# akio-tomiya/LatticeQCD.jl

Measured on AMD Instinct MI355X. Metric: CG iters/sec (D^+D) & Dslash GFLOP/s, 32^3x64 SU(3) Wilson fp64, higher is better.
Workload: dtype f64; 1 GPU; configs[3]: 32x32x32x64 Wilson D^+D CG (fixed-length window), fp64; dslash_variant=1, xcd_remap=2, xcd_nsub=16, xcd_ysplit=4, cg_fused=3, gauge_recon=12, gauge_recon_active=1, comm_backend=none, comm_requested=auto

## Files before the change

### latticeqcd.jl_amd/csrc/blas.hip

```cpp
#include "lqcd_internal.h"

#include <cstring>

namespace lqcd {

constexpr int RB = 256;

__device__ inline void block_reduce2(double a, double b, double* partial, int stride) {
    __shared__ double red[2][RB / 64];
#pragma unroll
    for (int off = 32; off > 0; off >>= 1) { a += __shfl_down(a, off, 64); b += __shfl_down(b, off, 64); }
    if ((threadIdx.x & 63) == 0) { red[0][threadIdx.x >> 6] = a; red[1][threadIdx.x >> 6] = b; }
    __syncthreads();
    if (threadIdx.x == 0) {
        double sa = 0, sb = 0;
#pragma unroll
        for (int w = 0; w < RB / 64; w++) { sa += red[0][w]; sb += red[1][w]; }
        partial[blockIdx.x * stride] = sa;
        if (stride > 1) partial[blockIdx.x * stride + 1] = sb;
    }
}

__global__ __launch_bounds__(RB) void dot_kernel(const double2* __restrict__ a, const double2* __restrict__ b, size_t n,
                                                 double* partial) {
    double re = 0, im = 0;
    for (size_t i = (size_t)blockIdx.x * RB + threadIdx.x; i < n; i += (size_t)gridDim.x * RB) {
        const double2 x = a[i], y = b[i];
        re = fma(x.x, y.x, re); re = fma(x.y, y.y, re);
        im = fma(x.x, y.y, im); im = fma(-x.y, y.x, im);
    }
    block_reduce2(re, im, partial, 2);
}

__global__ __launch_bounds__(RB) void norm2_kernel(const double2* __restrict__ a, size_t n, double* partial) {
    double s = 0;
    for (size_t i = (size_t)blockIdx.x * RB + threadIdx.x; i < n; i += (size_t)gridDim.x * RB) {
        const double2 x = a[i];
        s = fma(x.x, x.x, s); s = fma(x.y, x.y, s);
    }
    block_reduce2(s, 0.0, partial, 1);
}

__global__ __launch_bounds__(FB) void reduce_final(const double* __restrict__ partial, int nblocks, int nvals, double* scal, int slot, int op, PeerRedArgs pr, int soa) {
    __shared__ double tot[PEER_RED_VALS];
    if (nblocks <= 1024) {
        if (threadIdx.x < 64) {
            double mine = 0.0;
            for (int v = 0; v < nvals; v++) {
                const double t = sum_partials_small_nv(partial, nblocks, nvals, v, soa != 0);
                if (pr.nranks) { if (((int)threadIdx.x >> 3) == v) mine = t; }
                else if (threadIdx.x == 0) scal[slot + v] = t;
            }
            if (pr.nranks) {
                const double s = peer_allreduce_wave(pr, mine, nvals);
                for (int q = 0; q < nvals; q++) {
                    const double v = __shfl(s, 8 * q, 64);
                    if (threadIdx.x == 0) scal[slot + q] = v;
                }
            }
            if (op && threadIdx.x == 0) cg_scalar_step(scal, op);
        }
        return;
    }
    __shared__ double redv[PEER_RED_VALS][FB / 64];
    double cls[PEER_RED_VALS];
#pragma unroll
    for (int v = 0; v < PEER_RED_VALS; v++)
        if (v < nvals) cls[v] = sum_partials_class(partial, nblocks, nvals, v, (int)threadIdx.x, soa != 0);
#pragma unroll
    for (int v = 0; v < PEER_RED_VALS; v++)
        if (v < nvals) {
            const double w = shfl_tree_sum(cls[v]);
            if ((threadIdx.x & 63) == 0) redv[v][threadIdx.x >> 6] = w;
        }
    __syncthreads();
    if ((int)threadIdx.x < nvals) {
        double t = 0;
        for (int w = 0; w < FB / 64; w++) t += redv[threadIdx.x][w];
        if (pr.nranks) tot[threadIdx.x] = t; else scal[slot + threadIdx.x] = t;
    }
    __syncthreads();
    if (pr.nranks && threadIdx.x < 64) {
        const int k = (int)threadIdx.x >> 3;
        const double s = peer_allreduce_wave(pr, k < nvals ? tot[k] : 0.0, nvals);
        for (int q = 0; q < nvals; q++) {
            const double v = __shfl(s, 8 * q, 64);
            if (threadIdx.x == 0) scal[slot + q] = v;
        }
    }
    if (op && threadIdx.x == 0) cg_scalar_step(scal, op);
}

__global__ __launch_bounds__(RB) void axpy_kernel(double ar, double ai, const double2* __restrict__ x, double2* __restrict__ y, size_t n) {
    for (size_t i = (size_t)blockIdx.x * RB + threadIdx.x; i < n; i += (size_t)gridDim.x * RB) {
        const double2 xv = x[i];
        double2 yv = y[i];
        yv.x = fma(ar, xv.x, yv.x); yv.x = fma(-ai, xv.y, yv.x);
        yv.y = fma(ar, xv.y, yv.y); yv.y = fma(ai, xv.x, yv.y);
        y[i] = yv;
    }
}

__global__ __launch_bounds__(RB) void axpby_kernel(double ar, double ai, const double2* __restrict__ x, double br, double bi,
// ... 25 lines not shown
int allreduce_host(lqcd_ctx_s* c, double* vals, int n) {
    if (!c->has_comm) return LQCD_OK;
    ARGCHK(n <= 8, "allreduce_host: too many values");
    double* d = c->d_scal + SCAL_DOUBLES - 8;
    HIPCHK(hipMemcpyAsync(d, vals, n * sizeof(double), hipMemcpyHostToDevice, c->stream));
    LQCHK(comm_allreduce(c, d, n));
    HIPCHK(hipMemcpyAsync(vals, d, n * sizeof(double), hipMemcpyDeviceToHost, c->stream));
    HIPCHK(hipStreamSynchronize(c->stream));
    return comm_check(c);
}

int reduce_tail(lqcd_ctx_s* c, int nvals, int slot, int cg_op) {
    if (c->has_comm || cg_op) return comm_allreduce(c, c->d_scal + slot, nvals, cg_op);
    return LQCD_OK;
}

int reduce_to_slot(lqcd_ctx_s* c, int nblocks, int nvals, int slot, bool allreduce, int cg_op, const double* partial, bool soa) {
    const bool multi = allreduce && c->has_comm;
    const bool peer = multi && c->peer.on;
    ARGCHK(nvals >= 1 && nvals <= PEER_RED_VALS, "reduce_to_slot: one to eight values per reduction");
    if (peer) ARGCHK(nvals <= PEER_RED_VALS, "reduce_to_slot: more than 8 values in one reduction over the ranks");
    PeerRedArgs pr;
    if (peer) pr = comm_red_args(c); else memset(&pr, 0, sizeof pr);
    hipLaunchKernelGGL(reduce_final, dim3(1), dim3(FB), 0, c->stream, partial ? partial : c->d_partial, nblocks, nvals, c->d_scal, slot, (multi && !peer) ? 0 : cg_op, pr, soa ? 1 : 0);
    HIPCHK(hipGetLastError());
    if (multi && !peer) LQCHK(comm_allreduce(c, c->d_scal + slot, nvals, cg_op));
    return LQCD_OK;
}

int reduce_pack_to_slot(lqcd_ctx_s* c, int nblocks, int slot, int cg_op) {
    if (!c->has_waiting_pack) return reduce_to_slot(c, nblocks, 1, slot, true, cg_op);
    c->has_waiting_pack = false;
    const bool multi = c->has_comm, peer = multi && c->peer.on;
    LQCHK(launch_pack_reduce(c, *static_cast<StencilCall*>(c->waiting_pack), c->d_partial, nblocks, slot, (multi && !peer) ? 0 : cg_op));
    if (multi && !peer) LQCHK(comm_allreduce(c, c->d_scal + slot, 1, cg_op));
    return LQCD_OK;
}

static int fetch_slot(lqcd_ctx_s* c, int slot, int nvals, double* out) {
    HIPCHK(hipMemcpyAsync(c->h_scal, c->d_scal + slot, nvals * sizeof(double), hipMemcpyDeviceToHost, c->stream));
    HIPCHK(hipStreamSynchronize(c->stream));
    for (int i = 0; i < nvals; i++) out[i] = c->h_scal[i];
    return LQCD_OK;
}

int blas_dot(lqcd_ctx_s* c, const double2* a, const double2* b, size_t n, double* re, double* im, bool allreduce) {
    HIPCHK(hipSetDevice(c->device));
// ... 74 lines not shown
```

### latticeqcd.jl_amd/csrc/capi.hip

```cpp
#include "lqcd_internal.h"

#include <algorithm>
#include <cstdio>
#include <cstdlib>
#include <cstring>
#include <mutex>

namespace lqcd {

static thread_local std::string g_err;
static std::mutex g_live_mu;
static std::vector<const lqcd_ctx_s*> g_live;
bool ctx_is_live(const lqcd_ctx_s* c) {
    std::lock_guard<std::mutex> lk(g_live_mu);
    for (const lqcd_ctx_s* p : g_live)
        if (p == c) return true;
    return false;
}
static void ctx_set_live(const lqcd_ctx_s* c, bool live) {
    std::lock_guard<std::mutex> lk(g_live_mu);
    for (size_t i = 0; i < g_live.size(); i++)
        if (g_live[i] == c) { g_live.erase(g_live.begin() + i); break; }
    if (live) g_live.push_back(c);
}
// ... 155 lines not shown
    ARGCHK(V / 2 < (1ll << 31) / 16, "lqcd_ctx_create: local volume too large for 32-bit site indices");
    lqcd_ctx_s* c = new lqcd_ctx_s;
    c->home_thread = std::this_thread::get_id();
    c->device = device;
    c->rank = rank;
    c->nranks = pe[0] * pe[1] * pe[2] * pe[3];
    geom_from_L(c->geom, L);
    for (int mu = 0; mu < 4; mu++) {
        c->gL[mu] = gL[mu]; c->pe[mu] = pe[mu]; c->coord[mu] = coord[mu];
        c->nbr_fwd[mu] = nf[mu]; c->nbr_bwd[mu] = nb[mu];
        c->geom.gL[mu] = gL[mu]; c->geom.origin[mu] = origin[mu];
        c->geom.part[mu] = pe[mu] > 1 ? 1 : 0;
    }
    if (const char* e = getenv("LQCD_FORCE_PARTITION")) {
        const int mask = atoi(e);
        for (int mu = 0; mu < 4; mu++)
            if ((mask >> mu) & 1) c->geom.part[mu] = 1;
    }
    {
        const Geom& g = c->geom;
        const long slice = (long)g.XH * g.L[1] * g.L[2];
        if (slice % 64 == 0 && slice / 64 <= 128) { c->tun.xcd_nsub = 8; c->tun.xcd_ysplit = 2; }
        if (gauge12_elems(g) * sizeof(double2) <= ((size_t)256 << 20)) c->tun.nt_gauge = 0;
        if ((size_t)24 * g.Vh * sizeof(double2) <= ((size_t)64 << 20)) c->tun.nt_store = 0;
    }
    if (const char* e = getenv("LQCD_HALO_STREAM_MODE")) {
        const int v = atoi(e);
        if (v < -1 || v > 4) { set_error(std::string("LQCD_HALO_STREAM_MODE=") + e + ": the halo schedule is -1 (timed once) or 0..4"); delete c; return LQCD_ERR_ARG; }
        c->tun.halo_stream_mode = v;
    }
    if (const char* e = getenv("LQCD_HALO_FOLD")) {
        const int v = atoi(e);
        if (v != 0 && v != 1) { set_error(std::string("LQCD_HALO_FOLD=") + e + ": 0 or 1"); delete c; return LQCD_ERR_ARG; }
        c->tun.halo_fold = v;
    }
    hipDeviceProp_t prop;
    HIPCHK(hipGetDeviceProperties(&prop, device));
    c->num_cu = prop.multiProcessorCount > 0 ? prop.multiProcessorCount : 256;
    HIPCHK(hipStreamCreateWithFlags(&c->stream, hipStreamNonBlocking));
    HIPCHK(hipStreamCreateWithFlags(&c->comm_stream, hipStreamNonBlocking));
    HIPCHK(hipEventCreateWithFlags(&c->ev_pack, hipEventDisableTiming));
    HIPCHK(hipEventCreateWithFlags(&c->ev_comm, hipEventDisableTiming));
    HIPCHK(hipEventCreate(&c->ev_t0));
    HIPCHK(hipEventCreate(&c->ev_t1));
    HIPCHK(hipEventCreate(&c->ev_tune0));
    HIPCHK(hipEventCreate(&c->ev_tune1));
    const size_t npart = (size_t)2 * c->geom.Vh / 64 + 4096 + 8 * ((size_t)2 * c->geom.Vh / 128 + 8);
// ... 49 lines not shown
    (void)hipEventDestroy(c->ev_pack); (void)hipEventDestroy(c->ev_comm); (void)hipEventDestroy(c->ev_t0); (void)hipEventDestroy(c->ev_t1);
    (void)hipEventDestroy(c->ev_tune0); (void)hipEventDestroy(c->ev_tune1);
    (void)hipStreamDestroy(c->stream); (void)hipStreamDestroy(c->comm_stream);
    delete c;
    return LQCD_OK;
}

extern "C" int lqcd_ctx_sync(lqcd_ctx_t c) {
    ARGCHK(c, "lqcd_ctx_sync: null");
    LQCHK(ctx_drain_parked(c));
    LQCHK(links_flush_of(c));
    HIPCHK(hipSetDevice(c->device));
    HIPCHK(hipStreamSynchronize(c->stream));
    HIPCHK(hipStreamSynchronize(c->comm_stream));
    return comm_check(c);
}

static int* param_ptr(lqcd_ctx_s* c, const char* key) {
    if (!strcmp(key, "dslash_block")) return &c->tun.dslash_block;
    if (!strcmp(key, "xcd_remap")) return &c->tun.xcd_remap;
    if (!strcmp(key, "dslash_variant")) return &c->tun.dslash_variant;
    if (!strcmp(key, "nt_gauge")) return &c->tun.nt_gauge;
    if (!strcmp(key, "nt_store")) return &c->tun.nt_store;
    if (!strcmp(key, "cg_fused")) return &c->tun.cg_fused;
    if (!strcmp(key, "graph")) return &c->tun.graph;
    if (!strcmp(key, "gauge_recon")) return &c->tun.gauge_recon;
    if (!strcmp(key, "mixed_action_solver")) return &c->tun.mixed_action_solver;
    if (!strcmp(key, "mixed_pair32")) return &c->tun.mixed_pair32;
    if (!strcmp(key, "mixed_links16")) return &c->tun.mixed_links16;
    if (!strcmp(key, "bicg_reliable")) return &c->tun.bicg_reliable;
    if (!strcmp(key, "bicg_rec_guard")) return &c->tun.bicg_rec_guard;
    if (!strcmp(key, "bicg_dot_soa")) return &c->tun.bicg_dot_soa;
    if (!strcmp(key, "clover_hop_s")) return &c->tun.clover_hop_s;
    if (!strcmp(key, "mixed_lean_residual")) return &c->tun.mixed_lean_residual;
    if (!strcmp(key, "mixed_xfuse")) return &c->tun.mixed_xfuse;
    if (!strcmp(key, "mixed_defer_x")) return &c->tun.mixed_defer_x;
    if (!strcmp(key, "pair32_active")) return &c->tun.pair32_active;
    if (!strcmp(key, "stag_both")) return &c->tun.stag_both;
    if (!strcmp(key, "clover_fused")) return &c->tun.clover_fused;
    if (!strcmp(key, "clover_transport")) return &c->tun.clover_transport;
    if (!strcmp(key, "halo_stream_mode")) return &c->tun.halo_stream_mode;
    if (!strcmp(key, "cg_skip_done")) return &c->tun.cg_skip_done;
    if (!strcmp(key, "cg_small")) return &c->tun.cg_small;
    if (!strcmp(key, "cg_tgauge")) return &c->tun.cg_tgauge;
    if (!strcmp(key, "tgauge_active")) return &c->tun.tgauge_active;
    if (!strcmp(key, "cg_sweep_alt")) return &c->tun.cg_sweep_alt;
// ... 198 lines not shown
```

### latticeqcd.jl_amd/csrc/cg.hip

```cpp
#include "ops_internal.h"
#include "stencil_common.h"

#include <algorithm>
#include <cmath>

namespace lqcd {


__global__ void cg_scalar_alpha(double* s) {
    if (s[S_DONE] != 0.0) { s[S_XDONE] = 1.0; return; }
    s[S_ALPHA] = s[S_RR] / s[S_PQ];
}
__global__ void cg_scalar_beta(double* s) {
    if (s[S_DONE] != 0.0) return;
    const double rrn = s[S_RRNEW];
    s[S_BETA] = rrn / s[S_RR];
    s[S_RR] = rrn;
    s[S_ITERS] += 1.0;
    if (rrn < s[S_EPS]) s[S_DONE] = 1.0;
}

__global__ __launch_bounds__(UB) void cg_update_xr(const double* __restrict__ s, double2* __restrict__ x, double2* __restrict__ r,
                                                    const double2* __restrict__ p, const double2* __restrict__ q, size_t n,
                                                    double* partial) {
// ... 444 lines not shown
        apply_bc(c, op->bc);
        LQCHK(make_full_call(op, w.tmp, w.p, 0, s1));
        s1.skip_flag = c->tun.cg_skip_done ? c->d_scal : nullptr;
    } else {
        apply_bc(c, op->bc);
        LQCHK(make_full_call(op, w.tmp, rk, 0, s1));
        s1.upd_scal = c->d_scal;
        s1.upd[0] = spinor_block(w.tmp, 0);
        s1.upd[1] = spinor_block(w.tmp, 1);
        s1.upd_rec = 1;
    }
    s1.gauge12t = gt;
    s1.norm_partial = c->d_partial;
    LQCHK(stencil_apply(c, s1));
    LQCHK(reduce_to_slot(c, nbs, 1, S_PQ, true, m == 0 ? 9 : 7));
    apply_bc(c, op->bc);
    StencilCall s2;
    LQCHK(make_full_call(op, rn, w.tmp, 1, s2));
    s2.gauge12t = gt;
    s2.sweep_rev = w.sweep_alt ? 1 : 0;
    s2.norm_partial = c->d_partial;
    s2.upd_scal = c->d_scal;
    for (int q = 0; q < 2; q++) { s2.upd[q] = spinor_block(rn, q); s2.upd_src[q] = spinor_block(rk, q); }
    LQCHK(stencil_apply(c, s2));
    LQCHK(reduce_to_slot(c, nbs, 1, S_RRNEW, true, 8));
    w.k++;
    return LQCD_OK;
}
static int cg_rring_wanted(lqcd_op_s* op, const CgWork& w) {
    lqcd_ctx_s* c = op->ctx;
    const int K = c->tun.cg_rring;
    if (c->tun.cg_fused < 3 || !(K == 2 || K == 4 || K == 8)) return 0;
    if (op->kind != LQCD_WILSON || op->r != 1.0 || op->csw != 0.0 || any_partitioned(c) || c->has_comm || !c->local_peers.empty()) return 0;
    if (!stencil_sdir_applies(c, op->kind, op->r, op_fused_clover(op))) return 0;
    StencilCall s;
    if (make_full_call(op, w.tmp, w.p, 0, s) != LQCD_OK) return 0;
    if (!(w.tgauge || s.gauge12 || c->tun.dslash_s18)) return 0;
    return K;
}


static int cg_plain_tail(lqcd_ctx_s* c, double2* x, double2* r, double2* p, const double2* q, size_t n, bool dot_pq) {
    const int nb = stream_grid(c, n);
    if (dot_pq) {
        hipLaunchKernelGGL(redot_partial_kernel, dim3(nb), dim3(UB), 0, c->stream, p, q, n, c->d_partial);
        HIPCHK(hipGetLastError());
// ... 75 lines not shown
    const bool fp = part && defer && (c->tun.halo_fuse & 2) && op->kind == LQCD_WILSON && op->r == 1.0;
    {
        apply_bc(c, op->bc);
        StencilCall s1;
        LQCHK(make_full_call(op, w.tmp, pk, 0, s1));
        s1.gauge12t = gt;
        s1.norm_partial = c->d_partial;
        s1.skip_flag = c->tun.cg_skip_done ? c->d_scal : nullptr;
        if (fr) s1.red_slot = S_PQ;
        if (fp) { s1.pack_next = 1; s1.prepacked = (w.p_packed && w.pack_epoch == c->halo_epoch) ? 1 : 0; s1.defer_pack = folded ? 1 : 0; }
        LQCHK(stencil_apply(c, s1));
    }
    LQCHK(fr ? reduce_tail(c, 1, S_PQ, fold ? 0 : 1) : reduce_pack_to_slot(c, nbs, S_PQ, fold ? 0 : 1));
    apply_bc(c, op->bc);
    StencilCall s2;
    LQCHK(make_full_call(op, po, w.tmp, 1, s2));
    s2.gauge12t = gt;
    s2.sweep_rev = w.sweep_alt ? 1 : 0;
    s2.norm_partial = c->d_partial;
    if (fold) s2.scal_w = c->d_scal;
    s2.upd_scal = c->d_scal;
    s2.upd[0] = spinor_block(w.r, 0);
    s2.upd[1] = spinor_block(w.r, 1);
    if (fr) s2.red_slot = S_RRNEW;
    if (fp) s2.prepacked = 1;
    LQCHK(stencil_apply(c, s2));
    LQCHK(fr ? reduce_tail(c, 1, S_RRNEW, fold ? 0 : 2) : reduce_to_slot(c, nbs, 1, S_RRNEW, true, fold ? 0 : 2));
    const int nbu = stream_grid(c, n);
    HArgs h = HArgs();
    int npx = 0, npack = 0;
    if (fp) {
        int nt = 0;
        for (int mu = 0; mu < 4; mu++)
            if (c->geom.part[mu]) nt = std::max(nt, 2 * face_half_sites(c->geom, mu));
        npx = (nt + UB - 1) / UB; npack = 8 * npx;
        h.g = c->geom;
        h.gauge = op->gauge->data;
        h.parity_mode = 2; h.dagger = 0;
        for (int q = 0; q < 2; q++) { h.in[q] = spinor_block(pk, q); h.upd[q] = spinor_block(w.r, q); }
        for (int mu = 0; mu < 4; mu++) {
            const size_t cnt = (size_t)2 * 6 * face_half_sites(c->geom, mu);
            h.send_fwd[mu] = halo_send_base(c, mu, 0); h.send_bwd[mu] = halo_send_base(c, mu, 1) + cnt;
        }
    }
    const CgUpd u = {dim3(nbu + npack), x->data, pk->data, po->data, n, nbu, h, npx};
    if (!defer) hipLaunchKernelGGL(cg_update_xp, u.grid, dim3(UB), 0, c->stream, c->d_scal, x->data, w.p->data, w.r->data, n);
// ... 267 lines not shown
```

### latticeqcd.jl_amd/csrc/lqcd_internal.h

```cpp
#pragma once
#include <hip/hip_runtime.h>
#include <rccl/rccl.h>
#include <stdint.h>
#include <mutex>
#include <string>
#include <thread>
#include <vector>

#include "../../include/lqcd_hip.h"

namespace lqcd {

#ifdef LQCD_F32
typedef float real;
typedef float2 real2;
#define LQCD_PNS p32
inline namespace p32 {}
namespace p64 {}
#else
typedef double real;
typedef double2 real2;
#define LQCD_PNS p64
inline namespace p64 {}
namespace p32 {}
// ... 216 lines not shown
    double s0 = 0, s1 = 0, s2 = 0, s3 = 0;
    int i = cls;
    for (; i + 15 * FB < nblocks; i += 16 * FB) {
        double t[16];
#pragma unroll
        for (int k = 0; k < 16; k++) t[k] = partial[(size_t)(i + k * FB) * si];
#pragma unroll
        for (int q = 0; q < 4; q++) { s0 += t[4 * q]; s1 += t[4 * q + 1]; s2 += t[4 * q + 2]; s3 += t[4 * q + 3]; }
    }
    for (; i + 7 * FB < nblocks; i += 8 * FB) {
        double t[8];
#pragma unroll
        for (int k = 0; k < 8; k++) t[k] = partial[(size_t)(i + k * FB) * si];
#pragma unroll
        for (int q = 0; q < 2; q++) { s0 += t[4 * q]; s1 += t[4 * q + 1]; s2 += t[4 * q + 2]; s3 += t[4 * q + 3]; }
    }
    for (; i + 3 * FB < nblocks; i += 4 * FB) {
        s0 += partial[(size_t)i * si];
        s1 += partial[(size_t)(i + FB) * si];
        s2 += partial[(size_t)(i + 2 * FB) * si];
        s3 += partial[(size_t)(i + 3 * FB) * si];
    }
    for (; i < nblocks; i += FB) s0 += partial[(size_t)i * si];
    return (s0 + s1) + (s2 + s3);
}
__device__ inline double shfl_tree_sum(double s) {
#pragma unroll
    for (int off = 32; off > 0; off >>= 1) s += __shfl_down(s, off, 64);
    return s;
}

enum { S_RED0 = 0, S_RR = 8, S_PQ = 9, S_ALPHA = 10, S_BETA = 11, S_DONE = 12, S_ITERS = 13, S_EPS = 14, S_RRNEW = 15, S_XDONE = 16, S_RROLD = 17, S_APREV = 18,
       S_BSTART = 19,
       S_AHIST = 64,
       S_BHIST = 96,
       S_HIST_END = 128 };
constexpr int RRING_MAX = 32;
static_assert(S_BHIST - S_AHIST == RRING_MAX && S_HIST_END - S_BHIST == RRING_MAX && (RRING_MAX & (RRING_MAX - 1)) == 0, "the CG histories hold RRING_MAX entries each");
enum { B_RHO = 24, B_R0V = 26, B_VV = 28, B_ALPHA = 29, B_SS = 31, B_TS = 32, B_TT = 34, B_OMEGA = 35, B_RR = 37, B_RHO1 = 38, B_BETA = 40,
       B_DONE = 42, B_ITERS = 43, B_EPS = 44, B_HALF = 45, B_RES = 46, B_RHOB = 47, B_TS5 = 49, B_UNSURE = 54, B_XDONE = 55, B_END = 56 };
__device__ inline void cg_scalar_step(double* s, int op) {
    if (op == 1) {
        if (s[S_DONE] != 0.0) { s[S_XDONE] = 1.0; return; }
        s[S_ALPHA] = s[S_RR] / s[S_PQ];
    } else if (op == 2) {
        if (s[S_DONE] != 0.0) return;
// ... 26 lines not shown
            s[B_ALPHA + 1] = a.im;
        } else if (op == 4) {
            s[B_HALF] = (s[B_SS] < s[B_EPS]) ? 1.0 : 0.0;
        } else if (op == 5) {
            c2 ts = {s[B_TS], s[B_TS + 1]};
            const c2 w = bicg_omega(ts, s[B_TT], s[B_HALF] != 0.0);
            s[B_OMEGA] = w.re;
            s[B_OMEGA + 1] = w.im;
        } else {
            s[B_ITERS] += 1.0;
            const double rr = (s[B_HALF] != 0.0) ? s[B_SS] : s[B_RR];
            s[B_RES] = rr;
            if (s[B_HALF] != 0.0 || rr < s[B_EPS]) { s[B_DONE] = 1.0; return; }
            if (!(fabs(rr) <= 1.79e308)) { s[B_DONE] = 2.0; return; }
            c2 rho1 = {s[B_RHO1], s[B_RHO1 + 1]}, rho = {s[B_RHO], s[B_RHO + 1]}, al = {s[B_ALPHA], s[B_ALPHA + 1]}, om = {s[B_OMEGA], s[B_OMEGA + 1]};
            const c2 b = bicg_beta(rho1, rho, al, om);
            s[B_BETA] = b.re;
            s[B_BETA + 1] = b.im;
            s[B_RHO] = rho1.re; s[B_RHO + 1] = rho1.im;
        }
    }
}

__host__ __device__ inline uint64_t splitmix64(uint64_t x) {
    x += 0x9E3779B97F4A7C15ull;
    x = (x ^ (x >> 30)) * 0xBF58476D1CE4E5B9ull;
    x = (x ^ (x >> 27)) * 0x94D049BB133111EBull;
    return x ^ (x >> 31);
}
__host__ __device__ inline uint64_t rng_key(uint64_t seed, uint64_t site, uint64_t a, uint64_t b) {
    return splitmix64(splitmix64(splitmix64(seed ^ 0xA5A5A5A5DEADBEEFull) + site) + (a << 8) + b);
}
__host__ __device__ inline double u01(uint64_t k) { return ((k >> 11) + 0.5) * (1.0 / 9007199254740992.0); }

struct BlockMap {
    int nblocks, remap, cps, cpp, ysplit, cpr, ty, tz, LT;
    FastDiv d_perpass, d_cpr, d_ysplit, d_ty;
};
inline BlockMap make_block_map(const Geom& g, int remap, int nsub_in, int ysplit_in) {
    BlockMap m;
    const int TB = 64;
    const int chunks = (g.Vh + TB - 1) / TB;
    m.nblocks = 2 * chunks;
    m.remap = remap;
    m.LT = g.L[3];
    const int slice = g.XH * g.L[1] * g.L[2];
// ... 77 lines not shown
    int halo_fold = 1;
    int halo_fold_active = 0;
    int halo_fuse = 2;
    int cg_fold_scalars = 1;
    int nt_blas = 1;
    int md_reunitarize = 1;
    int staple_recon = 1;
    int staple_tile = 1;
    int md_remap = 1;
    int cg_defer_x = 1;
    int cg_persist = 1;
    int cg_small = 1;
    int cg_tgauge = 1;
    int tgauge_active = 0;
    int cg_sweep_alt = 1;
    int cg_sweep_alt_active = 0;
    int dslash_sweep = 0;
    int sweep_rev_active = 0;
    int dslash_xshare = 1;
    int xshare_active = 0;
    int dslash_yshare = 1;
    int yshare_active = 0;
    int nt_centre = 1;
    int cg_skip_done = 1;
    int clover_transport = 0;
    int stag_both = 0;
    int mixed_defer_x = 1;
    int mixed_xfuse = 0;
    int mixed_pair32 = 1;
    int mixed_action_solver = 0;
    int gauge_recon = 12;
#ifdef LQCD_VARIANTS
    int variants_built = 1;
#else
    int variants_built = 0;
#endif
    int bicg_fused = 4;
    int clover_hop_s = 1;
    int bicg_xrp_active = 0;
    int action_eo_solver = 1;
    int lazy_links = 0;
    int dw_batched = 1;
    int dw_fused_cg = 1;
    int dw_active = 0;
    int lazy_merge = 2;
    int mixed_lean_residual = 0;
// ... 342 lines not shown
PeerRedArgs comm_red_args(lqcd_ctx_s* c);
int comm_inject_stamp(lqcd_ctx_s* c, hipStream_t s);
int comm_inject_delay(lqcd_ctx_s* c, hipStream_t s);
int comm_check(lqcd_ctx_s* c);
void comm_teardown(lqcd_ctx_s* c);
double2* halo_send_base(lqcd_ctx_s* c, int mu, int toward_bwd);
const double2* halo_recv_base(lqcd_ctx_s* c, int mu);

struct StencilCall {
    int kind;
    const double2* gauge;
    double2* out[2];
    const double2* in[2];
    const double2* xin[2];
    double a, b;
    double r;
    int dagger;
    int parity_mode;
    double* norm_partial = nullptr;
    const double* upd_scal = nullptr;
    double2* upd[2] = {nullptr, nullptr};
    const double2* upd_src[2] = {nullptr, nullptr};
    int upd_rec = 0;
    int sweep_rev = 0;
    const double* skip_flag = nullptr;
    const double* alpha_partials = nullptr;
    int alpha_n = 0;
    double* scal_w = nullptr;
    const double2* gauge12 = nullptr;
    const double2* gauge12t = nullptr;
    const void* gauge16 = nullptr;
    int gauge12_delta = 0;
    const double2* clover = nullptr;
    int prec = 0;
    int red_slot = -1;
    int pack_next = -1;
    double2* xacc[2] = {nullptr, nullptr};
    const double2* pacc[2] = {nullptr, nullptr};
    int prepacked = 0;
    const double2* dot_z[2] = {nullptr, nullptr};
    double* dot_partial = nullptr;
    int dot_conj = 0;
    const double2* dot_z2[2] = {nullptr, nullptr};
    int dw_ls = 0;
    size_t dw_slice = 0;
    double dw_mass = 0.0;
// ... 104 lines not shown
```

### latticeqcd.jl_amd/csrc/stencil.hip

```cpp
#include "stencil_common.h"

#include <cstring>
namespace lqcd {
inline namespace LQCD_PNS {

template <int TB, bool DAG, bool RGEN>
__global__ __launch_bounds__(TB) void wilson_interior(KArgs k) {
    if (upd_done(k)) return;
    const real al_upd = update_alpha(k);
    int chunk, p;
    map_block(k, chunk, p);
    const int Vh = sp_stride(k.g);
    const int i = chunk * TB + threadIdx.x;
    const bool valid = i < k.g.Vh;
    real nrm = 0.0;
    if (valid) {
        Nbr n;
        int c[4];
        neighbours(k.g, p, i, n, c);
        cd acc[12], xv[12];
#pragma unroll
        for (int j = 0; j < 12; j++) acc[j] = mk(0.0, 0.0);
        if (k.a != 0.0) {
#pragma unroll
// ... 263 lines not shown


#ifndef LQCD_PIPE_DEARLY
#define LQCD_PIPE_DEARLY 0
#endif
#ifndef LQCD_PIPE_NOPF
#define LQCD_PIPE_NOPF 0
#endif
struct PipeArgs {
    const real2* gauge;
    const real2* clover;
    real2* dst[2];
    const real2* usrc[2];
    int rec;
    const real2* in[2];
    const real2* xin[2];
    double* norm_partial;
    const double* upd_scal;
    const double* skip;
    double* scal_w;
    real a, b;
    int nt_store;
    int nt_centre;
    int xshare;
    int yshare;
    int sweep_rev, nslab;
    int nvirt, both, pmode;
    int XH, L1, L2, LT, nch;
    FastDiv dXH;
    real sgn_f[4], sgn_b[4];
    int cps, cpp, cpr, per_pass, ty, tz, ysplit;
    FastDiv d_perpass, d_cpr, d_ysplit, d_ty, d_cpp;
    unsigned* ctr;
    int per_wg;
    const real2* dotz[2];
    const real2* dotz2[2];
    double* dot_partial;
    int dot_conj;
    int ls;
    unsigned long long slice_bytes;
    FastDiv d_ls;
    real dw_mass;
    int fold;
    int fsel;
    const int* vlist;
    const real2* gh_f[4];
// ... 726 lines not shown
        cd v = a.b * sm;
        v = mk(fma(a.a, xv[cc].re, v.re), fma(a.a, xv[cc].im, v.im));
        if constexpr (DW5) v = mk(v.re + w5[cc].re, v.im + w5[cc].im);
        if constexpr (DOT) {
            const cd z = z_is_x ? xv[cc] : rv[cc];
            nrm = fma(v.re, v.re, nrm); nrm = fma(v.im, v.im, nrm);
            if (a.nt_store) st_nt(dstp + co12(j), v); else st(dstp + co12(j), v);
            dre = fma(z.re, v.re, dre); dre = fma(z.im, v.im, dre);
            dim = fma(z.re, v.im, dim); dim = fma(-z.im, v.re, dim);
            if (two) {
                const cd z2 = rv[cc];
                dre2 = fma(z2.re, v.re, dre2); dre2 = fma(z2.im, v.im, dre2);
                dim2 = fma(z2.re, v.im, dim2); dim2 = fma(-z2.im, v.re, dim2);
            }
        } else if (a.upd_scal) {
            cd r = rv[cc];
            if (RING && a.rec) {
                r.re = fma(al_upd, r.re, v.re); r.im = fma(al_upd, r.im, v.im);
                nrm = fma(r.re, r.re, nrm); nrm = fma(r.im, r.im, nrm);
                if (a.nt_store) st_nt(dstp + co12(j), r); else st(dstp + co12(j), r);
            } else {
                r.re = fma(-al_upd, v.re, r.re); r.im = fma(-al_upd, v.im, r.im);
                nrm = fma(r.re, r.re, nrm); nrm = fma(r.im, r.im, nrm);
                st(dstp + co12(j), r);
            }
        } else {
            nrm = fma(v.re, v.re, nrm); nrm = fma(v.im, v.im, nrm);
            if (a.nt_store) st_nt(dstp + co12(j), v); else st(dstp + co12(j), v);
        }
    }
}

template <bool DAG, bool R12, bool NTB, bool DOT, bool DELTA, bool DW5, bool FOLD, bool CINV, bool TG>
__device__ __forceinline__ void dirsplit_s_block(const PipeArgs& a, real2 (*part)[12][64], double* red) {
    if ((a.upd_scal && a.upd_scal[S_DONE] != 0.0) || (a.skip && a.skip[S_DONE] != 0.0)) {
        if (a.scal_w && blockIdx.x == 0 && threadIdx.x == 0) a.scal_w[S_XDONE] = 1.0;
        return;
    }
    real al_upd = real(0);
    if (a.upd_scal) {
        if (!DOT && !DW5 && !FOLD && !CINV && a.rec) al_upd = (real)a.upd_scal[S_BETA];
        else if (a.scal_w) {
            const double rr = a.upd_scal[S_RR];
            const double al = rr / a.upd_scal[S_PQ];
            if (blockIdx.x == 0 && threadIdx.x == 0) { a.scal_w[S_ALPHA] = al; a.scal_w[S_RROLD] = rr; }
            al_upd = (real)al;
        } else al_upd = (real)a.upd_scal[S_ALPHA];
// ... 635 lines not shown
            if (s.dagger) hipLaunchKernelGGL((wilson_interior<TB, true, true>), grid, block, 0, c->stream, k);
            else hipLaunchKernelGGL((wilson_interior<TB, false, true>), grid, block, 0, c->stream, k);
        }
    } else {
        hipLaunchKernelGGL((staggered_interior<TB>), grid, block, 0, c->stream, k);
    }
    HIPCHK(hipGetLastError());
    return LQCD_OK;
}

static PipeArgs make_pipe_args(lqcd_ctx_s* c, const KArgs& k, const StencilCall& s) {
    PipeArgs a;
    a.gauge = k.gauge12 ? k.gauge12 : k.gauge;
    const bool upd = k.upd_scal != nullptr;
    for (int p = 0; p < 2; p++) { a.usrc[p] = s.upd_src[p] ? (const real2*)s.upd_src[p] : k.upd[p]; }
    a.rec = s.upd_rec;
    for (int p = 0; p < 2; p++) { a.dst[p] = upd ? k.upd[p] : k.out[p]; a.in[p] = k.in[p]; a.xin[p] = k.xin[p]; a.dotz[p] = k.dotz[p]; a.dotz2[p] = k.dotz2[p]; }
    a.dot_partial = k.dot_partial; a.dot_conj = k.dot_conj;
    a.clover = k.clover;
    a.norm_partial = k.norm_partial; a.upd_scal = k.upd_scal; a.skip = k.skip; a.scal_w = k.scal_w;
    a.a = k.a; a.b = k.b;
    a.nt_store = (k.nt & 4) != 0;
    a.nt_centre = c->tun.nt_centre != 0;
    a.xshare = 0; a.yshare = 0;
    a.sweep_rev = 0; a.nslab = 0;
    a.nvirt = k.nblocks; a.both = s.parity_mode == 2; a.pmode = s.parity_mode == 2 ? 0 : s.parity_mode;
    a.XH = k.g.XH; a.L1 = k.g.L[1]; a.L2 = k.g.L[2]; a.LT = k.g.L[3]; a.nch = k.g.nch; a.dXH = k.g.dXH;
    for (int mu = 0; mu < 4; mu++) {
        a.sgn_f[mu] = k.g.part[mu] ? real(0.0) : real(k.g.bc_fwd[mu]);
        a.sgn_b[mu] = k.g.part[mu] ? real(0.0) : real(k.g.bc_bwd[mu]);
    }
    a.cps = k.cps; a.cpp = k.cpp; a.cpr = k.cpr; a.per_pass = std::max(1, k.cpr * k.g.L[3]); a.ty = k.ty; a.tz = k.tz; a.ysplit = k.ysplit;
    a.ctr = c->pipe_ctr; a.per_wg = 1;
    a.d_perpass = k.d_perpass; a.d_cpr = k.d_cpr; a.d_ysplit = k.d_ysplit; a.d_ty = k.d_ty; a.d_cpp = make_fastdiv(std::max(1, k.cpp));
    a.ls = s.dw_ls; a.slice_bytes = (unsigned long long)s.dw_slice * sizeof(real2); a.d_ls = make_fastdiv(std::max(1, s.dw_ls)); a.dw_mass = (real)s.dw_mass;
    a.fold = 0;
    a.fsel = s.fold >= 2 ? s.fold - 1 : 0;
    a.vlist = nullptr;
    for (int mu = 0; mu < 4; mu++) {
        const size_t cnt = (size_t)(s.parity_mode == 2 ? 2 : 1) * 6 * face_half_sites(c->geom, mu);
        a.gh_b[mu] = (const real2*)halo_recv_base(c, mu); a.gh_f[mu] = (const real2*)halo_recv_base(c, mu) + cnt;
        a.Fh[mu] = face_half_sites(c->geom, mu);
        a.gsf[mu] = (c->coord[mu] == c->pe[mu] - 1) ? real(c->geom.bc_fwd[mu]) : real(1.0);
        a.gsb[mu] = (c->coord[mu] == 0) ? real(c->geom.bc_bwd[mu]) : real(1.0);
        if (s.fold && k.g.part[mu]) a.fold |= 1 << mu;
    }
// ... 188 lines not shown
#ifndef LQCD_F32
            if (k.gauge12 && c->tun.clover_hop_s && c->tun.dslash_pipe == 2 && !k.alpha_partials && !s.fold && wilson_pipe_applies(c, s.kind, s.r, s.parity_mode, false)) {
                PipeArgs a = make_pipe_args(c, k, s);
                const bool ntb = (k.nt & 1) != 0;
                if (s.dagger) { if (ntb) hipLaunchKernelGGL((wilson_dirsplit_s<true, true, true, false, false, false, false, true>), grid, block, 0, c->stream, a);
                                else hipLaunchKernelGGL((wilson_dirsplit_s<true, true, false, false, false, false, false, true>), grid, block, 0, c->stream, a); }
                else { if (ntb) hipLaunchKernelGGL((wilson_dirsplit_s<false, true, true, false, false, false, false, true>), grid, block, 0, c->stream, a);
                       else hipLaunchKernelGGL((wilson_dirsplit_s<false, true, false, false, false, false, false, true>), grid, block, 0, c->stream, a); }
            } else
#endif
            if (k.gauge12) { if (s.dagger) hipLaunchKernelGGL((wilson_dirsplit<true, true, false, false, true>), grid, block, pad, c->stream, k);
                             else hipLaunchKernelGGL((wilson_dirsplit<false, true, false, false, true>), grid, block, pad, c->stream, k); }
            else { if (s.dagger) hipLaunchKernelGGL((wilson_dirsplit<true, false, false, false, true>), grid, block, pad, c->stream, k);
                   else hipLaunchKernelGGL((wilson_dirsplit<false, false, false, false, true>), grid, block, pad, c->stream, k); }
        } else if (s.kind == LQCD_WILSON && !k.alpha_partials && wilson_pipe_applies(c, s.kind, s.r, s.parity_mode, k.clover != nullptr) &&
                   (c->tun.dslash_pipe != 2 || ((k.gauge12 || c->tun.dslash_s18) && !kF32Build))) {
            PipeArgs a = make_pipe_args(c, k, s);
            const bool persist = c->tun.dslash_pipe == 1 || c->tun.dslash_pipe == 3;
            if (c->tun.dslash_pipe == 3) { a.ctr = nullptr; a.per_wg = wilson_pipe_per_wg(c, k.nblocks); }
            const dim3 pg(c->tun.dslash_pipe == 1 ? wilson_pipe_grid(c, k.nblocks, s.prec) : c->tun.dslash_pipe == 3 ? k.nblocks / a.per_wg : k.nblocks), pb(256);
            const bool ntb = (k.nt & 1) != 0;
            pipe_sweep_args(c, k, s, delta, a);
            pipe_xshare_args(c, k, s, delta, a);
#ifndef LQCD_F32
            if (s.dw_ls > 1) {
                if (c->tun.dslash_pipe != 2 || delta) { set_error("stencil: the five-dimensional launch needs the scalar-addressing kernel in its plain mode"); return LQCD_ERR_UNSUPPORTED; }
                const dim3 g5((unsigned)k.nblocks * (unsigned)s.dw_ls);
                if (!k.gauge12) { set_error("stencil: the five-dimensional launch reads the 12-real links"); return LQCD_ERR_UNSUPPORTED; }
                if (s.dagger) hipLaunchKernelGGL((wilson_dirsplit_s<true, true, false, false, false, true>), g5, pb, 0, c->stream, a);
                else hipLaunchKernelGGL((wilson_dirsplit_s<false, true, false, false, false, true>), g5, pb, 0, c->stream, a);
            } else
            if (s.fold) {
                if (persist || delta || s.dw_ls > 1 || k.g.part[0]) { set_error("stencil: the folded launch needs the scalar-addressing kernel and an unpartitioned x direction"); return LQCD_ERR_UNSUPPORTED; }
                dim3 fg = pg;
                if (s.fold >= 2) {
                    int nb = 0;
                    LQCHK(fold_lists_get(c, 0, s, k, &a, &a.vlist, &nb));
                    if (nb == 0) return LQCD_OK;
                    fg = dim3(nb);
                }
#define LQ_FOLD(D, R) do { if (ntb) hipLaunchKernelGGL((wilson_dirsplit_s<D, R, true, false, false, false, true>), fg, pb, 0, c->stream, a); \
                           else hipLaunchKernelGGL((wilson_dirsplit_s<D, R, false, false, false, false, true>), fg, pb, 0, c->stream, a); } while (0)
                if (k.gauge12) { if (s.dagger) LQ_FOLD(true, true); else LQ_FOLD(false, true); }
                else { if (s.dagger) LQ_FOLD(true, false); else LQ_FOLD(false, false); }
#undef LQ_FOLD
            } else
// ... 193 lines not shown
```

Before: 1250 iter/s.

## Add nontemporal residual-update stores and prefetched CG scalar step in reductions

Adds an option to write the fused residual update in the Dslash pipe kernel with nontemporal stores, which is switched off for small lattices. Also adds a reduce_prefetch path that loads all partials up front and preloads the CG scalars so the alpha/beta step runs inside the reduction thread without a second pass. The prefetch path is off by default. For this 32^3x64 lattice the spinor is larger than 64MB, so nontemporal update stores stay enabled, which could free cache or could hurt if the residual is read back soon.

```diff
diff --git a/latticeqcd.jl_amd/csrc/blas.hip b/latticeqcd.jl_amd/csrc/blas.hip
--- a/latticeqcd.jl_amd/csrc/blas.hip
+++ b/latticeqcd.jl_amd/csrc/blas.hip
@@ -41,7 +41,7 @@
     block_reduce2(s, 0.0, partial, 1);
 }
 
-__global__ __launch_bounds__(FB) void reduce_final(const double* __restrict__ partial, int nblocks, int nvals, double* scal, int slot, int op, PeerRedArgs pr, int soa) {
+__global__ __launch_bounds__(FB) void reduce_final(const double* __restrict__ partial, int nblocks, int nvals, double* scal, int slot, int op, PeerRedArgs pr, int soa, int pf) {
     __shared__ double tot[PEER_RED_VALS];
     if (nblocks <= 1024) {
         if (threadIdx.x < 64) {
@@ -64,9 +64,19 @@
     }
     __shared__ double redv[PEER_RED_VALS][FB / 64];
     double cls[PEER_RED_VALS];
-#pragma unroll
-    for (int v = 0; v < PEER_RED_VALS; v++)
-        if (v < nvals) cls[v] = sum_partials_class(partial, nblocks, nvals, v, (int)threadIdx.x, soa != 0);
+    const bool step_pre = pf && op && nvals == 1 && !pr.nranks && cg_scalar_pre_applies(op, slot);
+    CgScalPre pre = {};
+    if (step_pre && threadIdx.x == 0) pre = cg_scalar_preload(scal);
+    if (pf && nvals == 1 && nblocks <= 32 * FB) cls[0] = sum_partials_class_all<32>(partial, nblocks, 1, 0, (int)threadIdx.x, soa != 0);
+    else if (pf && nblocks <= 4 * FB) {
+#pragma unroll
+        for (int v = 0; v < PEER_RED_VALS; v++)
+            if (v < nvals) cls[v] = sum_partials_class_all<4>(partial, nblocks, nvals, v, (int)threadIdx.x, soa != 0);
+    } else {
+#pragma unroll
+        for (int v = 0; v < PEER_RED_VALS; v++)
+            if (v < nvals) cls[v] = sum_partials_class(partial, nblocks, nvals, v, (int)threadIdx.x, soa != 0);
+    }
 #pragma unroll
     for (int v = 0; v < PEER_RED_VALS; v++)
         if (v < nvals) {
@@ -78,7 +88,9 @@
         double t = 0;
         for (int w = 0; w < FB / 64; w++) t += redv[threadIdx.x][w];
         if (pr.nranks) tot[threadIdx.x] = t; else scal[slot + threadIdx.x] = t;
-    }
+        if (step_pre) cg_scalar_step_pre(scal, op, pre, t);
+    }
+    if (step_pre) return;
     __syncthreads();
     if (pr.nranks && threadIdx.x < 64) {
         const int k = (int)threadIdx.x >> 3;
@@ -150,7 +162,7 @@
     if (peer) ARGCHK(nvals <= PEER_RED_VALS, "reduce_to_slot: more than 8 values in one reduction over the ranks");
     PeerRedArgs pr;
     if (peer) pr = comm_red_args(c); else memset(&pr, 0, sizeof pr);
-    hipLaunchKernelGGL(reduce_final, dim3(1), dim3(FB), 0, c->stream, partial ? partial : c->d_partial, nblocks, nvals, c->d_scal, slot, (multi && !peer) ? 0 : cg_op, pr, soa ? 1 : 0);
+    hipLaunchKernelGGL(reduce_final, dim3(1), dim3(FB), 0, c->stream, partial ? partial : c->d_partial, nblocks, nvals, c->d_scal, slot, (multi && !peer) ? 0 : cg_op, pr, soa ? 1 : 0, c->tun.reduce_prefetch ? 1 : 0);
     HIPCHK(hipGetLastError());
     if (multi && !peer) LQCHK(comm_allreduce(c, c->d_scal + slot, nvals, cg_op));
     return LQCD_OK;
diff --git a/latticeqcd.jl_amd/csrc/capi.hip b/latticeqcd.jl_amd/csrc/capi.hip
--- a/latticeqcd.jl_amd/csrc/capi.hip
+++ b/latticeqcd.jl_amd/csrc/capi.hip
@@ -201,7 +201,7 @@
         const long slice = (long)g.XH * g.L[1] * g.L[2];
         if (slice % 64 == 0 && slice / 64 <= 128) { c->tun.xcd_nsub = 8; c->tun.xcd_ysplit = 2; }
         if (gauge12_elems(g) * sizeof(double2) <= ((size_t)256 << 20)) c->tun.nt_gauge = 0;
-        if ((size_t)24 * g.Vh * sizeof(double2) <= ((size_t)64 << 20)) c->tun.nt_store = 0;
+        if ((size_t)24 * g.Vh * sizeof(double2) <= ((size_t)64 << 20)) { c->tun.nt_store = 0; c->tun.nt_upd_store = 0; }
     }
     if (const char* e = getenv("LQCD_HALO_STREAM_MODE")) {
         const int v = atoi(e);
@@ -297,6 +297,9 @@
     if (!strcmp(key, "dslash_variant")) return &c->tun.dslash_variant;
     if (!strcmp(key, "nt_gauge")) return &c->tun.nt_gauge;
     if (!strcmp(key, "nt_store")) return &c->tun.nt_store;
+    if (!strcmp(key, "nt_upd_store")) return &c->tun.nt_upd_store;
+    if (!strcmp(key, "upd_store_active")) return &c->tun.upd_store_active;
+    if (!strcmp(key, "reduce_prefetch")) return &c->tun.reduce_prefetch;
     if (!strcmp(key, "cg_fused")) return &c->tun.cg_fused;
     if (!strcmp(key, "graph")) return &c->tun.graph;
     if (!strcmp(key, "gauge_recon")) return &c->tun.gauge_recon;
diff --git a/latticeqcd.jl_amd/csrc/cg.hip b/latticeqcd.jl_amd/csrc/cg.hip
--- a/latticeqcd.jl_amd/csrc/cg.hip
+++ b/latticeqcd.jl_amd/csrc/cg.hip
@@ -490,6 +490,7 @@
     s2.norm_partial = c->d_partial;
     s2.upd_scal = c->d_scal;
     for (int q = 0; q < 2; q++) { s2.upd[q] = spinor_block(rn, q); s2.upd_src[q] = spinor_block(rk, q); }
+    s2.nt_upd = c->tun.nt_upd_store ? 1 : 0;
     LQCHK(stencil_apply(c, s2));
     LQCHK(reduce_to_slot(c, nbs, 1, S_RRNEW, true, 8));
     w.k++;
@@ -611,6 +612,7 @@
     s2.upd_scal = c->d_scal;
     s2.upd[0] = spinor_block(w.r, 0);
     s2.upd[1] = spinor_block(w.r, 1);
+    s2.nt_upd = (c->tun.nt_upd_store && !any_partitioned(c)) ? 1 : 0;
     if (fr) s2.red_slot = S_RRNEW;
     if (fp) s2.prepacked = 1;
     LQCHK(stencil_apply(c, s2));
diff --git a/latticeqcd.jl_amd/csrc/lqcd_internal.h b/latticeqcd.jl_amd/csrc/lqcd_internal.h
--- a/latticeqcd.jl_amd/csrc/lqcd_internal.h
+++ b/latticeqcd.jl_amd/csrc/lqcd_internal.h
@@ -262,6 +262,30 @@
         s3 += partial[(size_t)(i + 3 * FB) * si];
     }
     for (; i < nblocks; i += FB) s0 += partial[(size_t)i * si];
+    return (s0 + s1) + (s2 + s3);
+}
+template <int NMAX>
+__device__ inline double sum_partials_class_all(const double* __restrict__ partial, int nblocks, int nvals, int v, int cls, bool soa = false) {
+    const size_t si = soa ? 1 : (size_t)nvals;
+    partial += soa ? (size_t)v * nblocks : (size_t)v;
+    static_assert(NMAX % 4 == 0, "whole groups of four");
+    const int cnt = cls < nblocks ? (nblocks - cls + FB - 1) / FB : 0, c4 = cnt & ~3;
+    double t[NMAX];
+#pragma unroll
+    for (int k = 0; k < NMAX; k++) {
+        const int i = cls + k * FB;
+        t[k] = partial[(size_t)(i < nblocks ? i : nblocks - 1) * si];
+    }
+    double s0 = 0, s1 = 0, s2 = 0, s3 = 0;
+#pragma unroll
+    for (int k = 0; k < NMAX; k += 4) {
+        if (k < c4) { s0 += t[k]; s1 += t[k + 1]; s2 += t[k + 2]; s3 += t[k + 3]; }
+        else {
+#pragma unroll
+            for (int j = 0; j < 4; j++)
+                if (k + j < cnt) s0 += t[k + j];
+        }
+    }
     return (s0 + s1) + (s2 + s3);
 }
 __device__ inline double shfl_tree_sum(double s) {
@@ -334,6 +358,36 @@
     }
 }
 
+struct CgScalPre { double done, rr, iters, bstart, eps; };
+__device__ inline bool cg_scalar_pre_applies(int op, int slot) {
+    return ((op == 1 || op == 7 || op == 9) && slot == S_PQ) || ((op == 2 || op == 8) && slot == S_RRNEW);
+}
+__device__ inline CgScalPre cg_scalar_preload(const double* s) {
+    auto ldv = [&](int i) { return __hip_atomic_load(s + i, __ATOMIC_RELAXED, __HIP_MEMORY_SCOPE_AGENT); };
+    CgScalPre q;
+    q.done = ldv(S_DONE); q.rr = ldv(S_RR); q.iters = ldv(S_ITERS); q.bstart = ldv(S_BSTART); q.eps = ldv(S_EPS);
+    return q;
+}
+__device__ inline void cg_scalar_step_pre(double* s, int op, const CgScalPre& q_in, double red) {
+    CgScalPre q = q_in;
+    asm volatile("" : "+v"(q.done));
+    if (op == 1 || op == 7 || op == 9) {
+        if (q.done != 0.0) { s[S_XDONE] = 1.0; return; }
+        if (op == 9) s[S_BSTART] = q.iters;
+        const double al = q.rr / red;
+        s[S_ALPHA] = al;
+        if (op != 1) s[S_AHIST + ((int)(q.iters - (op == 9 ? q.iters : q.bstart)) & (RRING_MAX - 1))] = al;
+    } else {
+        if (q.done != 0.0) return;
+        const double be = red / q.rr;
+        s[S_BETA] = be;
+        if (op == 8) s[S_BHIST + ((int)(q.iters - q.bstart) & (RRING_MAX - 1))] = be;
+        s[S_RR] = red;
+        s[S_ITERS] = q.iters + 1.0;
+        if (red < q.eps) s[S_DONE] = 1.0;
+    }
+}
+
 __host__ __device__ inline uint64_t splitmix64(uint64_t x) {
     x += 0x9E3779B97F4A7C15ull;
     x = (x ^ (x >> 30)) * 0xBF58476D1CE4E5B9ull;
@@ -457,6 +511,9 @@
     int dslash_yshare = 1;
     int yshare_active = 0;
     int nt_centre = 1;
+    int nt_upd_store = 1;
+    int upd_store_active = 0;
+    int reduce_prefetch = 0;
     int cg_skip_done = 1;
     int clover_transport = 0;
     int stag_both = 0;
@@ -845,6 +902,7 @@
     double2* upd[2] = {nullptr, nullptr};
     const double2* upd_src[2] = {nullptr, nullptr};
     int upd_rec = 0;
+    int nt_upd = 0;
     int sweep_rev = 0;
     const double* skip_flag = nullptr;
     const double* alpha_partials = nullptr;
diff --git a/latticeqcd.jl_amd/csrc/stencil.hip b/latticeqcd.jl_amd/csrc/stencil.hip
--- a/latticeqcd.jl_amd/csrc/stencil.hip
+++ b/latticeqcd.jl_amd/csrc/stencil.hip
@@ -309,6 +309,7 @@
     real a, b;
     int nt_store;
     int nt_centre;
+    int nt_upd;
     int xshare;
     int yshare;
     int sweep_rev, nslab;
@@ -1081,7 +1082,7 @@
             } else {
                 r.re = fma(-al_upd, v.re, r.re); r.im = fma(-al_upd, v.im, r.im);
                 nrm = fma(r.re, r.re, nrm); nrm = fma(r.im, r.im, nrm);
-                st(dstp + co12(j), r);
+                if (RING && !kF32Build && a.nt_upd) st_nt(dstp + co12(j), r); else st(dstp + co12(j), r);
             }
         } else {
             nrm = fma(v.re, v.re, nrm); nrm = fma(v.im, v.im, nrm);
@@ -1763,6 +1764,7 @@
     a.a = k.a; a.b = k.b;
     a.nt_store = (k.nt & 4) != 0;
     a.nt_centre = c->tun.nt_centre != 0;
+    a.nt_upd = s.nt_upd ? 1 : 0;
     a.xshare = 0; a.yshare = 0;
     a.sweep_rev = 0; a.nslab = 0;
     a.nvirt = k.nblocks; a.both = s.parity_mode == 2; a.pmode = s.parity_mode == 2 ? 0 : s.parity_mode;
@@ -1997,6 +1999,10 @@
             const bool ntb = (k.nt & 1) != 0;
             pipe_sweep_args(c, k, s, delta, a);
             pipe_xshare_args(c, k, s, delta, a);
+            if (k.upd_scal && !s.upd_rec) {
+                if (kF32Build || persist || s.dw_ls > 1 || s.fold) a.nt_upd = 0;
+                c->tun.upd_store_active = a.nt_upd;
+            }
 #ifndef LQCD_F32
             if (s.dw_ls > 1) {
                 if (c->tun.dslash_pipe != 2 || delta) { set_error("stencil: the five-dimensional launch needs the scalar-addressing kernel in its plain mode"); return LQCD_ERR_UNSUPPORTED; }
```

After: 1246 iter/s, median of 2. No clear change (-0.4%).
